# ACMMM2021-Anonymous/video-graph-ssl

Hardware: AMD Instinct MI355X
Metric: pretrain_clips_per_sec (higher is better)
Workload: dtype bf16x6 (fp32 tensors; conv products as 6 bf16 MFMAs on hi/mid/lo splits = fp32-grade, fp32 accumulate; everything else fp32)

## Files before the change

### include/gca_hip.h

```cpp
#ifndef GCA_HIP_H
#define GCA_HIP_H

#include <stdint.h>

#ifdef __cplusplus
extern "C" {
#endif

#define GCA_OK 0
#define GCA_EINVAL (-1)
#define GCA_ELAUNCH (-2)

int gca_version(void);

int gca_conv_halo_occupancy(int tm, int tn, int math, int64_t lds_bytes);

int gca_set_conv_math(int mode);
int gca_get_conv_math(void);

typedef struct {
  int32_t N, C, D, H, W;
  int32_t K;
  int32_t kd, kh, kw;
  int32_t sd, sh, sw;
  int32_t pd, ph, pw;
  int32_t OD, OH, OW;
  int64_t x_batch_stride;
  int32_t tune_fwd_bm, tune_fwd_splits;
  int32_t tune_dgrad_bm, tune_dgrad_splits;
  int32_t tune_wgrad_splits, tune_wgrad_tile;
  int32_t tune_fwd_tail, tune_dgrad_tail;
  int32_t tune_fwd_math, tune_dgrad_math, tune_wgrad_math;
  int32_t tune_fwd_box, tune_dgrad_box;
// ... 1 lines not shown
} gca_conv_geom;

int64_t gca_conv_pack_elems(const gca_conv_geom* g, int which);
int gca_conv_pack(const gca_conv_geom* g, int which, const float* w, float* packed, void* stream);

#define GCA_PACK_JOB_BYTES 128
int64_t gca_conv_pack_jobs_host(const gca_conv_geom* g, int which, const float* w, float* packed, void* jobs_out);
int64_t gca_conv_pack_jobs_finalize_host(void* jobs, int64_t njobs);
int gca_conv_pack_batched(const void* jobs_dev, int64_t njobs, int64_t total_blocks, void* stream);

int64_t gca_conv_table_rows(const gca_conv_geom* g, int which);
int gca_conv_table_build_host(const gca_conv_geom* g, int which, int32_t* table_host );

int64_t gca_conv_fwd_stat_parts(const gca_conv_geom* g);
int gca_conv_kernel_cfg(const gca_conv_geom* g, int which, int32_t* out4);
int64_t gca_conv_pack_layout(const gca_conv_geom* g, int which);
int64_t gca_conv_fwd_ws_bytes(const gca_conv_geom* g);
int gca_conv_fwd(const gca_conv_geom* g, const void* x, const float* wpack, const int32_t* table,
                 const float* bias, void* y, float* stat_sum, float* stat_sq, void* ws, void* stream);

int64_t gca_conv_dgrad_ws_bytes(const gca_conv_geom* g);
int gca_conv_dgrad(const gca_conv_geom* g, const void* dy, const float* wpack, const int32_t* table,
                   void* dx, int accumulate, void* ws, void* stream);

int64_t gca_conv_wgrad_ws_bytes(const gca_conv_geom* g);
int gca_conv_wgrad(const gca_conv_geom* g, const void* x, const void* dy, const int32_t* table,
                   float* dw, int accumulate, void* ws, void* stream);
typedef struct {
  const float* slabs;
  float* dw;
// ... 164 lines not shown
```

### video-graph-ssl_amd/_hip.py

```python
import ctypes as C
import os

import torch

_HERE = os.path.dirname(os.path.abspath(__file__))
LIB_PATH = os.environ.get('GCA_LIB_PATH') or os.path.join(_HERE, 'libgca_hip.so')


class HipLibraryMissing(RuntimeError):
    pass


if not os.path.exists(LIB_PATH):
    raise HipLibraryMissing(
        'libgca_hip.so is not built (%s). Run ./build_hip.sh or __graft_entry__.build(); there is no '
        'CPU fallback for the product path.' % LIB_PATH)
lib = C.CDLL(LIB_PATH)

c_i32, c_i64, c_f32, c_f64, c_vp = C.c_int32, C.c_int64, C.c_float, C.c_double, C.c_void_p


class ConvGeom(C.Structure):
    _fields_ = [(n, c_i32) for n in ('N', 'C', 'D', 'H', 'W', 'K', 'kd', 'kh', 'kw', 'sd', 'sh', 'sw',
                                     'pd', 'ph', 'pw', 'OD', 'OH', 'OW')] + [('x_batch_stride', c_i64)] + \
# ... 2 lines not shown
                                     'tune_fwd_math', 'tune_dgrad_math', 'tune_wgrad_math', 'tune_fwd_box',
                                     'tune_dgrad_box', 'act_f16')]


class PoolGeom(C.Structure):
    _fields_ = [(n, c_i32) for n in ('N', 'C', 'D', 'H', 'W', 'kd', 'kh', 'kw', 'sd', 'sh', 'sw',
                                     'pd', 'ph', 'pw', 'OD', 'OH', 'OW')]


_GP, _PP = C.POINTER(ConvGeom), C.POINTER(PoolGeom)
SIGNATURES = {
    'gca_version': (c_i32, []),
    'gca_conv_halo_occupancy': (c_i32, [c_i32, c_i32, c_i32, c_i64]),
    'gca_set_conv_math': (c_i32, [c_i32]),
    'gca_get_conv_math': (c_i32, []),
    'gca_conv_pack_elems': (c_i64, [_GP, c_i32]),
    'gca_conv_pack': (c_i32, [_GP, c_i32, c_vp, c_vp, c_vp]),
    'gca_conv_table_rows': (c_i64, [_GP, c_i32]),
    'gca_conv_table_build_host': (c_i32, [_GP, c_i32, c_vp]),
    'gca_conv_fwd_stat_parts': (c_i64, [_GP]),
    'gca_conv_kernel_cfg': (c_i32, [_GP, c_i32, c_vp]),
    'gca_conv_pack_layout': (c_i64, [_GP, c_i32]),
    'gca_conv_fwd_ws_bytes': (c_i64, [_GP]),
    'gca_conv_fwd': (c_i32, [_GP, c_vp, c_vp, c_vp, c_vp, c_vp, c_vp, c_vp, c_vp, c_vp]),
    'gca_conv_dgrad_ws_bytes': (c_i64, [_GP]),
    'gca_conv_dgrad': (c_i32, [_GP, c_vp, c_vp, c_vp, c_vp, c_i32, c_vp, c_vp]),
    'gca_conv_wgrad_cfg': (c_i32, [_GP, c_vp]),
    'gca_conv_wgrad_ws_bytes': (c_i64, [_GP]),
    'gca_conv_wgrad': (c_i32, [_GP, c_vp, c_vp, c_vp, c_vp, c_i32, c_vp, c_vp]),
    'gca_bias_grad': (c_i32, [c_vp, c_i64, c_i64, c_i64, c_vp, c_i32, c_vp]),
    'gca_bn_stats': (c_i32, [c_vp, c_i64, c_i64, c_i64, c_vp, c_vp, c_vp, c_i32, c_vp]),
    'gca_bn_stats_parts': (c_i64, [c_i64, c_i64, c_i64]),
    'gca_bn_finalize': (c_i32, [c_vp, c_vp, c_i64, c_i64, c_f64, c_vp, c_vp, c_f32, c_f32, c_vp, c_vp, c_vp,
                                c_vp, c_vp, c_vp, c_vp, c_vp]),
    'gca_bn_train_fwd': (c_i32, [c_vp, c_vp, c_i64, c_i64, c_f64, c_vp, c_vp, c_f32, c_f32, c_vp, c_vp, c_vp,
                                 c_vp, c_vp, c_vp, c_vp, c_vp, c_vp, c_i32, c_i64, c_i64, c_vp, c_i64, c_i32, c_vp]),
# ... 123 lines not shown
```

### video-graph-ssl_amd/csrc/conv3d.hip

```cpp
#include <cstring>
#include <type_traits>
#include "conv_halo.h"

#include <cstdlib>
#include <vector>

using namespace gca_conv;

namespace {


constexpr int LDK = BK + 4;
constexpr int lds_pitch(int math) { return math == 2 ? 28 : (math == 3 ? 12 : LDK); }
constexpr int lds_bufs(int tm, bool vec, int math) { return (math >= 1 || vec || tm >= 4) ? 1 : 2; }
constexpr int cmax(int a, int b) { return a > b ? a : b; }

template <int TM, int BN, int FAST, bool VEC, int MATH, bool H = false>
__device__ __forceinline__ void igemm_tile(
    const void* __restrict__ src, const float* __restrict__ apack, const int2* __restrict__ table,
    const float* __restrict__ bias, void* __restrict__ dst, float* __restrict__ psum,
    float* __restrict__ psq, float* __restrict__ slab, const IgemmParams p, int bid,
    float* __restrict__ As_, float* __restrict__ Bs_, int* __restrict__ taptab) {
  constexpr unsigned ES = H ? 2u : 4u;
  constexpr int BM = 32 * TM, TN = BN / 128;
// ... 765 lines not shown
  pw.accumulate = ip.accumulate;
  pw.src_nstride = (unsigned)ip.src_nstride;
  pw.src_bytes = ip.src_bytes; pw.dst_bytes = ip.dst_bytes;
  const long long pb = (long long)pack_rows(DK) * pw.Kpad * 2;
  pw.pack_bytes = clamp_buf_bytes(pb);
  return true;
}

inline int stem_copy_dwords(int bw) { return (bw + 4) / 2; }
inline int stem_row_bytes(int bw, int sh, int np) { (void)sh; return 4 * np * stem_copy_dwords(bw) * 4; }
inline bool stem_heuristic_on() {
  static int on = -1;
  if (on < 0) { const char* e = getenv("GCA_STEM"); on = (e && e[0] == '0') ? 0 : 1; }
  return on != 0;
}
inline bool stem_geometry(const gca_conv_geom* g, const IgemmParams& p, int math, StemParams& sp) {
  if (math < 1 || math > 3 || g->C > 4 || g->sw != 2 || g->kw > 8 || g->x_batch_stride % 4 != 0) return false;
  if ((long long)g->N * g->OD * g->OH * g->OW < 256 * 32) return false;
  const int np = math == 3 ? 1 : (math == 2 ? 3 : 2);
  const int nrows = g->C * g->kd * g->kh, nsteps = cdiv(nrows, 2);
  double best = 1e300;
  int bb[3] = {0, 0, 0};
  const int wmr = g->K > 64 ? 4 : 2, npos = 512 / wmr;
  for (int pass = 0; pass < 2 && bb[0] == 0; ++pass) {
    const size_t cap = pass == 0 ? (size_t)(76 << 10) : (size_t)(156 << 10);
    for (int bd = 1; bd <= npos; bd *= 2)
      for (int bh = 1; bd * bh <= npos; bh *= 2) {
        const int bw = npos / (bd * bh);
        if (bw < 4 || bw > 64) continue;
        if (bd > 2 * g->OD || bh > 2 * g->OH || bw > 2 * g->OW) continue;
        const int hd = (bd - 1) * g->sd + g->kd, hh = (bh - 1) * g->sh + g->kh, wp = bw + 4;
        const size_t lds = gca_round_up((2 * nsteps + g->C * hd * hh) * 4, 16) + (size_t)g->C * hd * hh * stem_row_bytes(bw, g->sh, np);
        if (lds > cap) continue;
        const double cover = (double)cdiv(g->OD, bd) * bd / g->OD * cdiv(g->OH, bh) * bh / g->OH * cdiv(g->OW, bw) * bw / g->OW;
        const double staging = (double)g->C * hd * hh * 2 * wp / (double)npos;
        const double cost = cover * (1.0 + staging / (double)(nsteps * 8)) * (bw >= 8 ? 1.0 : 1.15);
        if (cost < best) { best = cost; bb[0] = bd; bb[1] = bh; bb[2] = bw; }
      }
  }
  if (bb[0] == 0) return false;
  sp.g = p;
  sp.wm = wmr;
  sp.bd = bb[0]; sp.bh = bb[1]; sp.bw = bb[2]; sp.lbh = ilog2(bb[1]); sp.lbw = ilog2(bb[2]);
  sp.nbd = cdiv(g->OD, sp.bd); sp.nbh = cdiv(g->OH, sp.bh); sp.nbw = cdiv(g->OW, sp.bw);
  sp.hd = (sp.bd - 1) * g->sd + g->kd; sp.hh = (sp.bh - 1) * g->sh + g->kh; sp.wp = sp.bw + 4;
  sp.cd = stem_copy_dwords(sp.bw); sp.hrowb = stem_row_bytes(sp.bw, g->sh, np);
  sp.sd = g->sd; sp.sh = g->sh; sp.pd = g->pd; sp.ph = g->ph; sp.pw = g->pw;
  sp.kd = g->kd; sp.kh = g->kh; sp.kw = g->kw;
  sp.nrows = nrows; sp.nsteps = nsteps;
  sp.Mrows = pack_rows(g->K);
  sp.rowoff_bytes = (int)gca_round_up((2 * nsteps + g->C * sp.hd * sp.hh) * 4, 16);
  sp.cs_bytes = (unsigned)((long long)g->D * g->H * g->W * (g->act_f16 ? 2 : 4));
  const long long pb = (long long)nsteps * sp.Mrows * (math == 3 ? 32 : (math == 2 ? 96 : 64));
  sp.pack_bytes = clamp_buf_bytes(pb);
  sp.m_w2 = gca_make_magic((unsigned)sp.wp); sp.m_hdh = gca_make_magic((unsigned)(sp.hd * sp.hh));
  sp.m_hh = gca_make_magic((unsigned)sp.hh);
  return true;
// ... 46 lines not shown
                           ((double)c.q[0] * c.q[1] * c.q[2]);
      const double cost = cover * (1.0 + 0.08 * hp.P / bn) * (w >= 8 ? 1.0 : (w >= 4 ? 1.1 : 1.3));
      if (cost < best) { best = cost; bd = d; bh = h; bw = w; }
    }
  cost_out = best;
  return best < 1e299;
}

inline IgemmCfg cfg_for(const gca_conv_geom* g, int which, const ClassInfo& c, const IgemmParams& p, size_t nclasses) {
  int fbm, fs, tail, box;
  tune_of(g, which, fbm, fs, tail, box);
  const int math = resolve_math(which == 0 ? g->tune_fwd_math : g->tune_dgrad_math, g->act_f16);
  if (which == 0 && ((fbm & 4096) || (fbm == 0 && stem_heuristic_on()))) {
    StemParams sp;
    if (stem_geometry(g, p, math, sp))
      return IgemmCfg{32 * sp.wm, 512 / sp.wm, 1, sp.nsteps, 0, 0, math, ConvKernel::Stem, sp.bd, sp.bh, sp.bw, math == 3};
  }
  if (fbm & 4096) { fbm = 0; fs = 0; tail = 0; }
  if ((fbm & 8192) || (fbm == 0 && pw_heuristic_on())) {
    PwParams pw;
    if (pw_geometry(g, which, p, pw)) return IgemmCfg{128, 128, 1, pw.Kpad / 32, 0, 0, 3, ConvKernel::Pointwise, 0, 0, 0, 1};
  }
  if (fbm & 8192) { fbm = 0; fs = 0; tail = 0; }
  {
    int bd = box & 255, bh = (box >> 8) & 255, bw = (box >> 16) & 255, rows = fbm & 1023;
    bool use = false;
    HaloParams hp;
    if ((fbm & 2048) && !(fbm & (4096 | 8192))) {
      use = bd > 0 && halo_geometry(c, p, bd, bh, bw, math, hp);
    } else if (fbm == 0 && halo_heuristic_on() && (c.ntaps >= 3 || math == 3) && c.srcC >= 32 && p.Ntot >= 128LL * 192) {
      double cost = 0, cost2 = 0;
// ... 54 lines not shown
  else
    hipLaunchKernelGGL((conv_igemm_kernel<TM, BN, FAST, VEC, 0>), grid, dim3(256), 0, st, src, apack, table, bias,
                       dst, psum, psq, slab, p);
}

template <int TM>
void launch_tm(const IgemmCfg& c, int fast, dim3 grid, hipStream_t st, const float* src, const float* apack,
               const int2* table, const float* bias, float* dst, float* psum, float* psq, float* slab,
               const IgemmParams& p) {
  if (c.bn == 256) launch_one<TM, 256, 1, true>(c.math, grid, st, src, apack, table, bias, dst, psum, psq, slab, p, c.h);
  else if (fast == 1) launch_one<TM, 128, 1, false>(c.math, grid, st, src, apack, table, bias, dst, psum, psq, slab, p, c.h);
  else if (fast == 2) launch_one<TM, 128, 2, false>(c.math, grid, st, src, apack, table, bias, dst, psum, psq, slab, p, c.h);
  else launch_one<TM, 128, 0, false>(c.math, grid, st, src, apack, table, bias, dst, psum, psq, slab, p, c.h);
}

inline int stat_parts(const IgemmCfg& c, long long Ntot, long long halo_tiles = 0) {
  if (c.splits > 1) return (int)gca_ceil_div(Ntot, FINISH_CHUNK);
  if (c.kernel != ConvKernel::Gather) return (int)halo_tiles;
  return (int)gca_ceil_div(Ntot, c.bn);
}

int finish_slabs(const IgemmCfg& c, const float* slab, const float* bias, float* dst, float* psum, float* psq, const IgemmParams& p,
                 hipStream_t st) {
  const dim3 grid((unsigned)p.DK, (unsigned)p.P);
  if (c.h)
    hipLaunchKernelGGL(conv_splitk_finish_kernel<_Float16>, grid, dim3(256), 0, st, slab, c.splits, bias,
                       reinterpret_cast<_Float16*>(dst), psum, psq, p);
  else
    hipLaunchKernelGGL(conv_splitk_finish_kernel<float>, grid, dim3(256), 0, st, slab, c.splits, bias, dst, psum, psq, p);
  return gca_launch_status();
}

// ... 78 lines not shown
  return finish_slabs(cf, slab, bias, dst, psum, psq, p, st);
}

int run_class_pw(const gca_conv_geom* g, int which, const float* src, const float* apack, const float* bias, float* dst, float* psum,
                 float* psq, const IgemmParams& p, hipStream_t st) {
  PwParams pw;
  if (!pw_geometry(g, which, p, pw)) return GCA_EINVAL;
  return pw_launch(pw, src, reinterpret_cast<const unsigned char*>(apack), bias, dst, psum, psq, st);
}

int run_class_stem(const gca_conv_geom* g, const IgemmCfg& cf, const float* src, const float* apack, const float* bias, float* dst,
                   float* psum, float* psq, const IgemmParams& p, hipStream_t st) {
  StemParams sp;
  if (!stem_geometry(g, p, cf.math, sp) || sp.bd != cf.bd || sp.bh != cf.bh || sp.bw != cf.bw) return GCA_EINVAL;
  sp.g.splits = 1; sp.g.kt_per_split = sp.nsteps;
  sp.g.tilesM = cdiv(p.DK, 32 * sp.wm);
  const long long tn = (long long)g->N * sp.nbd * sp.nbh * sp.nbw;
  if (tn > 0x7fffffffLL) return GCA_EINVAL;
  sp.g.tilesN = (int)tn; sp.g.tileN_off = 0;
  sp.g.P = (int)tn;
  return stem_launch(cf.math, sp, src, reinterpret_cast<const unsigned char*>(apack), bias, dst, psum, psq, st);
}

struct ConvLaunch {
  std::vector<ClassInfo> cls;
  std::vector<IgemmParams> p;
  std::vector<IgemmCfg> cf;
};

ConvLaunch resolve_launch(const gca_conv_geom* g, int which) {
  ConvLaunch L;
  build_classes(g, which, L.cls);
  const size_t n = L.cls.size();
  L.p.assign(n, IgemmParams{});
  L.cf.assign(n, IgemmCfg{});
// ... 42 lines not shown
  }
  return g_conv_math;
}
}

extern "C" {

int gca_version(void) { return 15; }

int gca_set_conv_math(int mode) {
  if (mode < 0 || mode > 2) return GCA_EINVAL;
  g_conv_math = mode;
  return GCA_OK;
}
int gca_get_conv_math(void) { return conv_math(); }

int64_t gca_conv_pack_elems(const gca_conv_geom* g, int which) {
  if (!geom_ok(g) || (which != 0 && which != 1)) return GCA_EINVAL;
  int64_t n = 0;
  for (const ClassInfo& c : resolve_launch(g, which).cls) n += pack_reserve(c);
  return n > 0 ? n : 64;
}

static void pack_params_of(const gca_conv_geom* g, int which, const ClassInfo& c, const IgemmCfg& cf, PackParams& p) {
  const int T = taps(g);
  p.fmt = (int)cf.kernel; p.math = cf.math; p.SC = c.srcC;
  p.nsteps = cf.kernel == ConvKernel::Stem ? cf.kt_per_split : cdiv(c.srcC, 16) * c.ntaps;
  const bool pwfmt = p.fmt == 3;
  p.Kred = (int)c.Kred; p.M = c.M; p.Kpad = pwfmt ? (int)gca_round_up(c.srcC, 32) : (int)c.Kpad; p.Mrows = pack_rows(c.M);
  p.ntaps = p.fmt == 2 ? g->kd * g->kh : c.ntaps; p.nb = c.nb; p.nc = c.nc;
// ... 142 lines not shown
int gca_conv_kernel_cfg(const gca_conv_geom* g, int which, int32_t* out4) {
  if (!geom_ok(g) || which < 0 || which > 1 || !out4) return GCA_EINVAL;
  const ConvLaunch L = resolve_launch(g, which);
  for (size_t i = 0; i < L.cls.size(); ++i) {
    const ClassInfo& c = L.cls[i];
    const IgemmCfg& cf = L.cf[i];
    if (c.ntaps == 0) continue;
    out4[0] = cf.bm; out4[1] = cf.bn; out4[2] = cf.splits;
    out4[3] = (int)L.cls.size() | (fast_of(c.ntaps) << 8) | (c.vec << 10) | (cf.math << 12) | ((cf.kernel == ConvKernel::Halo) << 14) |
              (cf.h << 15) | ((cf.kernel == ConvKernel::Stem) << 16) | ((cf.kernel == ConvKernel::Pointwise) << 17);
    return GCA_OK;
  }
  return GCA_EINVAL;
}

int64_t gca_conv_fwd_stat_parts(const gca_conv_geom* g) {
  if (!geom_ok(g)) return GCA_EINVAL;
  const ConvLaunch L = resolve_launch(g, 0);
  const IgemmCfg& cf = L.cf[0];
  if (cf.kernel == ConvKernel::Pointwise) return (int64_t)g->N * cdiv((int)((long long)g->OD * g->OH * g->OW), 128);
  return stat_parts(cf, L.p[0].Ntot, cf.kernel != ConvKernel::Gather ? halo_tiles_n(g, L.cls[0], cf) : 0);
}

int64_t gca_conv_fwd_ws_bytes(const gca_conv_geom* g) { return geom_ok(g) ? ws_bytes_for(g, 0) : GCA_EINVAL; }
int64_t gca_conv_dgrad_ws_bytes(const gca_conv_geom* g) { return geom_ok(g) ? ws_bytes_for(g, 1) : GCA_EINVAL; }

int gca_conv_fwd(const gca_conv_geom* g, const void* x_, const float* wpack, const int32_t* table,
                 const float* bias, void* y_, float* stat_sum, float* stat_sq, void* ws, void* stream) {
  const float* x = reinterpret_cast<const float*>(x_);
  float* y = reinterpret_cast<float*>(y_);
// ... 70 lines not shown
```

### video-graph-ssl_amd/csrc/conv3d_stem.hip

```cpp
#include <cstring>
#include "conv_igemm_host.h"
#include "conv_halo.h"

using namespace gca_conv;

namespace {

constexpr int rowb(int math) { return math == 3 ? 32 : (math == 2 ? 96 : 64); }
constexpr int nparts(int math) { return math == 3 ? 1 : (math == 2 ? 3 : 2); }
__device__ __forceinline__ unsigned short f16_bits(float v) { return __builtin_bit_cast(unsigned short, (_Float16)v); }

template <int MATH, int WM>
__global__ __launch_bounds__(256, 2) void conv_stem_kernel(
    const void* __restrict__ src, const unsigned char* __restrict__ apack, const float* __restrict__ bias,
    void* __restrict__ dst, float* __restrict__ psum, float* __restrict__ psq, const StemParams sp) {
  static_assert(MATH >= 1 && MATH <= 3, "bf16x3 / bf16x6 / fp16 storage");
  constexpr bool F16 = MATH == 3;
  constexpr unsigned ES = F16 ? 2u : 4u;
  static_assert(WM == 2 || WM == 4, "wave grid");
  constexpr int WN = 4 / WM, BM = 32 * WM, TN = 4;
  constexpr int ROWB = rowb(MATH), NP = nparts(MATH);
  const IgemmParams& p = sp.g;
  extern __shared__ __attribute__((aligned(16))) unsigned char smem[];
  int* const rowoff = reinterpret_cast<int*>(smem);
  unsigned* const rowbase = reinterpret_cast<unsigned*>(smem) + 2 * sp.nsteps;
  unsigned char* const Hs = smem + sp.rowoff_bytes;

  const int tid = threadIdx.x, lane = tid & 63, wave = tid >> 6, wm = wave / WN, wn = wave % WN, lh = lane >> 5, ll = lane & 31;
  int bid = gca_xcd_remap(blockIdx.x, gridDim.x);
  const int tileM = bid % p.tilesM, tileN = bid / p.tilesM;
  const int per_img = sp.nbd * sp.nbh * sp.nbw;
  const int img = tileN / per_img;
  int tb = tileN - img * per_img;
  const int tbd = tb / (sp.nbh * sp.nbw); tb -= tbd * (sp.nbh * sp.nbw);
  const int tbh = tb / sp.nbw, tbw = tb - tbh * sp.nbw;
  const int q0d = tbd * sp.bd, q0h = tbh * sp.bh, q0w = tbw * sp.bw;

  const int wp = sp.wp;
  const unsigned COPYB = (unsigned)sp.cd * 4u, PARTB = 2u * COPYB, PHASEB = PARTB * NP, HROWB = (unsigned)sp.hrowb;
  const int khd = sp.kd * sp.kh;
  for (int r = tid; r < 2 * sp.nsteps; r += 256) {
    int off = 0;
    if (r < sp.nrows) {
      const int c = r / khd, ab = r - c * khd, a = ab / sp.kh, b = ab - a * sp.kh;
      off = ((c * sp.hd + a) * sp.hh + b) * (int)HROWB;
    }
    rowoff[r] = off;
  }

  const __amdgpu_buffer_rsrc_t ra = __builtin_amdgcn_make_buffer_rsrc(const_cast<unsigned char*>(apack), 0, sp.pack_bytes, 0x00020000);
  const unsigned avoff = (unsigned)(tileM * BM + 32 * wm + ll) * ROWB + (unsigned)lh * 16u;
  const unsigned astep = (unsigned)sp.Mrows * ROWB;
  float4 afn[NP];
  auto a_issue = [&](int s) __attribute__((always_inline)) {
#pragma unroll
    for (int q = 0; q < NP; ++q) {
      const f32x4 f = __builtin_bit_cast(f32x4, __builtin_amdgcn_raw_buffer_load_b128(ra, (int)(avoff + 32u * q), (int)((unsigned)s * astep), 0));
      afn[q] = make_float4(f.x, f.y, f.z, f.w);
    }
  };
  a_issue(0);

  {
    const __amdgpu_buffer_rsrc_t rs = __builtin_amdgcn_make_buffer_rsrc(const_cast<void*>(src), 0, p.src_bytes, 0x00020000);
    const int nhrows = p.SC * sp.hd * sp.hh;
    const int s0d = q0d * sp.sd - sp.pd, s0h = q0h * sp.sh - sp.ph, s0w = q0w * 2 - sp.pw;
    const unsigned ibase = (unsigned)((long long)img * p.src_nstride);
    const int hdh = sp.hd * sp.hh;
    for (int hr = tid; hr < nhrows; hr += 256) {
      const int c = (int)gca_fdiv((unsigned)hr, sp.m_hdh), rem = hr - c * hdh;
      const int zd = (int)gca_fdiv((unsigned)rem, sp.m_hh), zh = rem - zd * sp.hh;
      const int id = s0d + zd, ih = s0h + zh;
      const bool ok = (unsigned)id < (unsigned)p.SD && (unsigned)ih < (unsigned)p.SH;
      rowbase[hr] = ok ? (ibase + (unsigned)((id * p.SH + ih) * p.SW)) * ES + (unsigned)c * sp.cs_bytes : 0xffffffffu;
    }
// ... 39 lines not shown
          unsigned h, l;
          split_bf16x2(v[k][0], v[k][1], h, l);
          *reinterpret_cast<unsigned*>(d) = h; *reinterpret_cast<unsigned*>(d + PARTB) = l;
          split_bf16x2(v[k][1], v[k][2], h, l);
          *reinterpret_cast<unsigned*>(d + COPYB) = h; *reinterpret_cast<unsigned*>(d + COPYB + PARTB) = l;
        }
      }
    }
  }

  unsigned bpos[TN];
  bool cval[TN];
  int cq[TN][3];
#pragma unroll
  for (int j = 0; j < TN; ++j) {
    const int cidx = wn * 128 + j * 32 + ll;
    const int zw = cidx & (sp.bw - 1), t1 = cidx >> sp.lbw;
    const int zh = t1 & (sp.bh - 1), zd = t1 >> sp.lbh;
    cq[j][0] = q0d + zd; cq[j][1] = q0h + zh; cq[j][2] = q0w + zw;
    cval[j] = cq[j][0] < p.QD && cq[j][1] < p.QH && cq[j][2] < p.QW;
    bpos[j] = (unsigned)((zd * sp.sd) * sp.hh + zh * sp.sh) * HROWB + (unsigned)(zw & 1) * COPYB + (unsigned)(zw & ~1) * 2u;
  }

  f32x16 acc[TN];
#pragma unroll
  for (int j = 0; j < TN; ++j)
#pragma unroll
    for (int r = 0; r < 16; ++r) acc[j][r] = 0.f;

  auto load_b = [&](float4 (&bf)[NP], int j, unsigned ro) __attribute__((always_inline)) {
    const unsigned char* bp = Hs + bpos[j] + ro;
#pragma unroll
    for (int q = 0; q < NP; ++q) {
      const unsigned* e = reinterpret_cast<const unsigned*>(bp + q * PARTB);
      const unsigned* o = reinterpret_cast<const unsigned*>(bp + PHASEB + q * PARTB);
      bf[q] = make_float4(__uint_as_float(e[0]), __uint_as_float(e[1]), __uint_as_float(o[0]), __uint_as_float(o[1]));
    }
  };
  auto mma = [&](f32x16& c, const float4 (&af)[NP], const float4 (&bf)[NP]) __attribute__((always_inline)) {
    if constexpr (MATH == 3) {
      c = __builtin_amdgcn_mfma_f32_32x32x16_f16(__builtin_bit_cast(f16x8, af[0]), __builtin_bit_cast(f16x8, bf[0]), c, 0, 0, 0);
    } else {
      const bf16x8 xh = __builtin_bit_cast(bf16x8, af[0]), xl = __builtin_bit_cast(bf16x8, af[NP - 1]);
// ... 7 lines not shown
        c = __builtin_amdgcn_mfma_f32_32x32x16_bf16(xh, ym, c, 0, 0, 0);
      } else {
        c = __builtin_amdgcn_mfma_f32_32x32x16_bf16(xl, yh, c, 0, 0, 0);
        c = __builtin_amdgcn_mfma_f32_32x32x16_bf16(xh, yl, c, 0, 0, 0);
      }
      c = __builtin_amdgcn_mfma_f32_32x32x16_bf16(xh, yh, c, 0, 0, 0);
    }
  };

  __syncthreads();
  unsigned ro = (unsigned)rowoff[lh];
  float4 bfc[NP], bfn[NP];
  load_b(bfc, 0, ro);
  for (int s = 0; s < sp.nsteps; ++s) {
    const unsigned ro_next = (unsigned)rowoff[2 * min(s + 1, sp.nsteps - 1) + lh];
    float4 af[NP];
#pragma unroll
    for (int q = 0; q < NP; ++q) af[q] = afn[q];
    a_issue(min(s + 1, sp.nsteps - 1));
#pragma unroll
    for (int j = 0; j < TN; ++j) {
      if (j + 1 < TN) load_b(bfn, j + 1, ro); else load_b(bfn, 0, ro_next);
      mma(acc[j], af, bfc);
#pragma unroll
      for (int q = 0; q < NP; ++q) bfc[q] = bfn[q];
    }
    ro = ro_next;
  }
  __syncthreads();

  const int mbase = tileM * BM + 32 * wm;
  const int rows_left = p.DK - mbase - 4 * lh;
  const int DHW = p.DH * p.DW;
  const unsigned DSP = (unsigned)(p.DD * DHW);
  const unsigned rowb_ = DSP * ES;
  const __amdgpu_buffer_rsrc_t rd = __builtin_amdgcn_make_buffer_rsrc(dst, 0, p.dst_bytes, 0x00020000);
#pragma unroll
  for (int j = 0; j < TN; ++j) {
    const unsigned dsp = (unsigned)(cq[j][0] * DHW + cq[j][1] * p.DW + cq[j][2]);
    const unsigned vb = cval[j] ? (((unsigned)img * (unsigned)p.DK + (unsigned)(mbase + 4 * lh)) * DSP + dsp) * ES : 0xffffffffu;
#pragma unroll
    for (int r = 0; r < 16; ++r) {
      const int rr = (r & 3) + 8 * (r >> 2);
      const unsigned vo = rr < rows_left ? vb : 0xffffffffu;
      float v = acc[j][r];
      if (bias) v += bias[min(mbase + rr + 4 * lh, p.DK - 1)];
      if (F16) __builtin_amdgcn_raw_buffer_store_b16(f16_bits(v), rd, (int)vo, (int)((unsigned)rr * rowb_), 0);
      else __builtin_amdgcn_raw_buffer_store_b32(__float_as_uint(v), rd, (int)vo, (int)((unsigned)rr * rowb_), 0);
    }
  }
  if (psum) {
    float* red = reinterpret_cast<float*>(Hs);
#pragma unroll
    for (int r = 0; r < 16; ++r) {
      float sm = 0.f, sq = 0.f;
#pragma unroll
      for (int j = 0; j < TN; ++j) { const float v = cval[j] ? acc[j][r] : 0.f; sm += v; sq += v * v; }
      sm = half_wave_sum_hi(sm);
      sq = half_wave_sum_hi(sq);
      const int rr = 32 * wm + (r & 3) + 8 * (r >> 2) + 4 * lh;
      if (ll == 31) { red[(wn * BM + rr) * 2] = sm; red[(wn * BM + rr) * 2 + 1] = sq; }
    }
    __syncthreads();
    if (tid < BM && tileM * BM + tid < p.DK) {
      float sm = red[tid * 2], sq = red[tid * 2 + 1];
      if (WN == 2) { sm += red[(BM + tid) * 2]; sq += red[(BM + tid) * 2 + 1]; }
      const long long m = tileM * BM + tid;
      psum[m * p.P + tileN] = sm;
      psq[m * p.P + tileN] = sq;
    }
  }
}

}

namespace gca_conv {

size_t stem_lds_bytes(const StemParams& sp, int math) {
  const size_t halo = (size_t)sp.g.SC * sp.hd * sp.hh * sp.hrowb;
  return (size_t)sp.rowoff_bytes + (halo > 2048 ? halo : 2048);
}

int stem_launch(int math, const StemParams& sp, const void* src, const unsigned char* apack, const float* bias, void* dst,
                float* psum, float* psq, hipStream_t st) {
  const size_t lds = stem_lds_bytes(sp, math);
  const long long nblk = (long long)sp.g.tilesM * sp.g.tilesN;
  if (nblk <= 0 || nblk > 0x7fffffffLL || lds > (size_t)(160 << 10) - 1024) return GCA_EINVAL;
  static bool raised[4][2] = {};
#define GCA_SK2(M, W)                                                                                                      \
  {                                                                                                                        \
    if (lds > (48u << 10) && !raised[M][W / 4]) {                                                                          \
      if (hipFuncSetAttribute(reinterpret_cast<const void*>(&conv_stem_kernel<M, W>),                                      \
                              hipFuncAttributeMaxDynamicSharedMemorySize, 160 << 10) != hipSuccess) return GCA_ELAUNCH;   \
      raised[M][W / 4] = true;                                                                                             \
    }                                                                                                                      \
    hipLaunchKernelGGL((conv_stem_kernel<M, W>), dim3((unsigned)nblk), dim3(256), lds, st, src, apack, bias, dst, psum, psq, sp); \
  }
#define GCA_SK(M) { if (sp.wm == 4) GCA_SK2(M, 4) else GCA_SK2(M, 2) }
  switch (math) {
    case 1: GCA_SK(1) break;
    case 2: GCA_SK(2) break;
    case 3: GCA_SK(3) break;
    default: return GCA_EINVAL;
  }
#undef GCA_SK
#undef GCA_SK2
  return gca_launch_status();
}

}
```

### video-graph-ssl_amd/csrc/conv_halo.h

```cpp
#pragma once
#include "conv_igemm_host.h"

namespace gca_conv {

struct HaloParams {
  IgemmParams g;
  int bd, bh, bw;
  int lbh, lbw;
  int hd, hh, hw;
  int h0d, h0h, h0w;
  int dmin_d, dmin_h, dmin_w;
  int nbd, nbh, nbw;
  int P;
  int nchunks, chunks_per_split;
  int Mrows;
  unsigned cs_bytes;
  unsigned pack_bytes;
  const float* in_scale;
  const float* in_shift;
};

struct HaloCfg {
  int bm, bn;
  int bd, bh, bw;
  int splits, chunks_per_split;
  int math;
};

struct StemParams {
  IgemmParams g;
  int wm;
  int bd, bh, bw, lbh, lbw;
  int nbd, nbh, nbw;
  int hd, hh;
  int wp;
  int cd, hrowb;
  int sd, sh, pd, ph, pw;
  int kd, kh, kw;
  int nrows, nsteps;
  int Mrows;
  int rowoff_bytes;
  unsigned cs_bytes;
  unsigned pack_bytes;
  gca_magic m_w2, m_hdh, m_hh;
};

// ... 85 lines not shown
```

### video-graph-ssl_amd/engine/ops.py

```python
import ctypes as C
import functools
import os

import torch

from .. import _hip as H
from .._hip import aptr, is_half, ptr, stream
from . import tune
from .tune import TUNE_HALO, TUNE_PW, TUNE_STEM, TUNE_VEC

F32 = torch.float32
F16 = torch.float16


def _t3(v):
    return (v, v, v) if isinstance(v, int) else tuple(int(a) for a in v)


class _Workspace:

    def __init__(self):
        self.buf = {}
        self.captured = set()
        self.retired = []
# ... 26 lines not shown
_TUNE_DIRTY = [False]
_TUNE_PATH = os.environ.get('GCA_TUNE_CACHE', '')


CONV_MATH = {'f32': 0, 'bf16x3': 1, 'bf16x6': 2}
ACT_F16 = [False]


def set_conv_math(mode):
    ACT_F16[0] = mode == 'fp16'
    H.call('gca_set_conv_math', CONV_MATH['bf16x6' if mode == 'fp16' else mode])


def get_conv_math():
    return 'fp16' if ACT_F16[0] else ('f32', 'bf16x3', 'bf16x6')[H.lib.gca_get_conv_math()]


def cast_f16(x):
    rows, re = (1, x.numel()) if x.is_contiguous() else (x.shape[0], x[0].numel())
    if not x.is_contiguous() and not x[0].is_contiguous():
        raise RuntimeError('only channel slices of a contiguous (N, Ctot, ...) buffer are supported')
    y = torch.empty(x.shape, dtype=F16, device=x.device)
    H.call('gca_cast_f16', ptr(x), rows, re, re if x.is_contiguous() else x.stride(0), aptr(y), stream())
    return y


def load_tune_cache(path):
    import json
    with open(path) as f:
        for k, v in json.load(f).items():
# ... 75 lines not shown
        out = (C.c_int32 * 4)()
        if which == 2:
            H.call('gca_conv_wgrad_cfg', self.gp, out)
        else:
            H.call('gca_conv_kernel_cfg', self.gp, which, out)
        return tuple(out)

    WGRAD_KERNELS = {11: 'temporal32', 12: 'temporal64', 13: 'spatial', 14: 'stem'}
    WGRAD_SHAPES = tune.WGRAD_SHAPES

    def kernel(self, which):
        kc = self.cfg(which)[3]
        if which == 2:
            return self.WGRAD_KERNELS.get(kc & 255, 'gather')
        return next((name for name, _, bit in _KERNELS if kc >> bit & 1), 'gather')

    def math(self, which):
        return self.cfg(which)[3] >> 12 & 3

    def pack_layout(self, which):
        return 0 if which == 2 else H.lib.gca_conv_pack_layout(self.gp, which)

    def tune_key(self, which):
        g = self.g
        geom = (g.N, g.C, g.D, g.H, g.W, g.K, g.kd, g.kh, g.kw, g.sd, g.sh, g.sw, g.pd, g.ph, g.pw, g.x_batch_stride)
        return 'v%d%s:%d:%s' % (H.lib.gca_version(), 'h' if g.act_f16 else ('', 'b', 'c')[H.lib.gca_get_conv_math()], which,
                                ','.join(str(int(v)) for v in geom))

    def set_code(self, which, code):
        for field, v in zip(code._fields, code):
# ... 700 lines not shown
```

Baseline: 1670.

## Add register-blocked stem conv tile computing two M sub-tiles per wave

Adds an RT=2 variant of the stem conv kernel where each wave holds two 32-row M sub-tiles of accumulators and reuses each loaded B fragment for two MFMAs. For bf16x6 with K>64 it uses WM=2,RT=2 over 256 positions, and for fp16 it uses WM=1,RT=2. This halves B-fragment LDS reads per MFMA. BN-stat partial reduction is reworked to match, with per-half partials and an LDS exchange. It is enabled by default through GCA_STEM_RB, and it raises register pressure and changes the stat-part count layout.

```diff
diff --git a/include/gca_hip.h b/include/gca_hip.h
--- a/include/gca_hip.h
+++ b/include/gca_hip.h
@@ -17,6 +17,9 @@
 
 int gca_set_conv_math(int mode);
 int gca_get_conv_math(void);
+
+int gca_set_stem_rb(int on);
+int gca_get_stem_rb(void);
 
 typedef struct {
   int32_t N, C, D, H, W;
@@ -48,6 +51,7 @@
 
 int64_t gca_conv_fwd_stat_parts(const gca_conv_geom* g);
 int gca_conv_kernel_cfg(const gca_conv_geom* g, int which, int32_t* out4);
+int gca_conv_stem_shape(const gca_conv_geom* g, int32_t* out4);
 int64_t gca_conv_pack_layout(const gca_conv_geom* g, int which);
 int64_t gca_conv_fwd_ws_bytes(const gca_conv_geom* g);
 int gca_conv_fwd(const gca_conv_geom* g, const void* x, const float* wpack, const int32_t* table,
diff --git a/video-graph-ssl_amd/_hip.py b/video-graph-ssl_amd/_hip.py
--- a/video-graph-ssl_amd/_hip.py
+++ b/video-graph-ssl_amd/_hip.py
@@ -40,12 +40,15 @@
     'gca_conv_halo_occupancy': (c_i32, [c_i32, c_i32, c_i32, c_i64]),
     'gca_set_conv_math': (c_i32, [c_i32]),
     'gca_get_conv_math': (c_i32, []),
+    'gca_set_stem_rb': (c_i32, [c_i32]),
+    'gca_get_stem_rb': (c_i32, []),
     'gca_conv_pack_elems': (c_i64, [_GP, c_i32]),
     'gca_conv_pack': (c_i32, [_GP, c_i32, c_vp, c_vp, c_vp]),
     'gca_conv_table_rows': (c_i64, [_GP, c_i32]),
     'gca_conv_table_build_host': (c_i32, [_GP, c_i32, c_vp]),
     'gca_conv_fwd_stat_parts': (c_i64, [_GP]),
     'gca_conv_kernel_cfg': (c_i32, [_GP, c_i32, c_vp]),
+    'gca_conv_stem_shape': (c_i32, [_GP, c_vp]),
     'gca_conv_pack_layout': (c_i64, [_GP, c_i32]),
     'gca_conv_fwd_ws_bytes': (c_i64, [_GP]),
     'gca_conv_fwd': (c_i32, [_GP, c_vp, c_vp, c_vp, c_vp, c_vp, c_vp, c_vp, c_vp, c_vp]),
diff --git a/video-graph-ssl_amd/csrc/conv3d.hip b/video-graph-ssl_amd/csrc/conv3d.hip
--- a/video-graph-ssl_amd/csrc/conv3d.hip
+++ b/video-graph-ssl_amd/csrc/conv3d.hip
@@ -803,33 +803,48 @@
   if (on < 0) { const char* e = getenv("GCA_STEM"); on = (e && e[0] == '0') ? 0 : 1; }
   return on != 0;
 }
+int g_stem_rb = -1;
+inline bool stem_rb_on() {
+  if (g_stem_rb < 0) { const char* e = getenv("GCA_STEM_RB"); g_stem_rb = (e && e[0] == '0') ? 0 : 1; }
+  return g_stem_rb != 0;
+}
+inline bool stem_pick_box(const gca_conv_geom* g, int npos, int np, int nsteps, size_t cap, int (&bb)[3]) {
+  double best = 1e300;
+  bb[0] = 0;
+  for (int bd = 1; bd <= npos; bd *= 2)
+    for (int bh = 1; bd * bh <= npos; bh *= 2) {
+      const int bw = npos / (bd * bh);
+      if (bw < 4 || bw > 64) continue;
+      if (bd > 2 * g->OD || bh > 2 * g->OH || bw > 2 * g->OW) continue;
+      const int hd = (bd - 1) * g->sd + g->kd, hh = (bh - 1) * g->sh + g->kh, wp = bw + 4;
+      const size_t lds = gca_round_up((2 * nsteps + g->C * hd * hh) * 4, 16) + (size_t)g->C * hd * hh * stem_row_bytes(bw, g->sh, np);
+      if (lds > cap) continue;
+      const double cover = (double)cdiv(g->OD, bd) * bd / g->OD * cdiv(g->OH, bh) * bh / g->OH * cdiv(g->OW, bw) * bw / g->OW;
+      const double staging = (double)g->C * hd * hh * 2 * wp / (double)npos;
+      const double cost = cover * (1.0 + staging / (double)(nsteps * 8)) * (bw >= 8 ? 1.0 : 1.15);
+      if (cost < best) { best = cost; bb[0] = bd; bb[1] = bh; bb[2] = bw; }
+    }
+  return bb[0] != 0;
+}
 inline bool stem_geometry(const gca_conv_geom* g, const IgemmParams& p, int math, StemParams& sp) {
   if (math < 1 || math > 3 || g->C > 4 || g->sw != 2 || g->kw > 8 || g->x_batch_stride % 4 != 0) return false;
   if ((long long)g->N * g->OD * g->OH * g->OW < 256 * 32) return false;
   const int np = math == 3 ? 1 : (math == 2 ? 3 : 2);
   const int nrows = g->C * g->kd * g->kh, nsteps = cdiv(nrows, 2);
-  double best = 1e300;
   int bb[3] = {0, 0, 0};
-  const int wmr = g->K > 64 ? 4 : 2, npos = 512 / wmr;
-  for (int pass = 0; pass < 2 && bb[0] == 0; ++pass) {
-    const size_t cap = pass == 0 ? (size_t)(76 << 10) : (size_t)(156 << 10);
-    for (int bd = 1; bd <= npos; bd *= 2)
-      for (int bh = 1; bd * bh <= npos; bh *= 2) {
-        const int bw = npos / (bd * bh);
-        if (bw < 4 || bw > 64) continue;
-        if (bd > 2 * g->OD || bh > 2 * g->OH || bw > 2 * g->OW) continue;
-        const int hd = (bd - 1) * g->sd + g->kd, hh = (bh - 1) * g->sh + g->kh, wp = bw + 4;
-        const size_t lds = gca_round_up((2 * nsteps + g->C * hd * hh) * 4, 16) + (size_t)g->C * hd * hh * stem_row_bytes(bw, g->sh, np);
-        if (lds > cap) continue;
-        const double cover = (double)cdiv(g->OD, bd) * bd / g->OD * cdiv(g->OH, bh) * bh / g->OH * cdiv(g->OW, bw) * bw / g->OW;
-        const double staging = (double)g->C * hd * hh * 2 * wp / (double)npos;
-        const double cost = cover * (1.0 + staging / (double)(nsteps * 8)) * (bw >= 8 ? 1.0 : 1.15);
-        if (cost < best) { best = cost; bb[0] = bd; bb[1] = bh; bb[2] = bw; }
-      }
-  }
-  if (bb[0] == 0) return false;
+  const bool rb = stem_rb_on();
+  int wmr = g->K > 64 ? 4 : 2, rt = 1;
+  if (g->K > 64) {
+    if (rb && math == 2 && stem_pick_box(g, 256, np, nsteps, (size_t)(76 << 10), bb)) { wmr = 2; rt = 2; }
+    else if (!stem_pick_box(g, 128, np, nsteps, (size_t)(76 << 10), bb) && !stem_pick_box(g, 128, np, nsteps, (size_t)(156 << 10), bb))
+      return false;
+  } else {
+    if (!stem_pick_box(g, 256, np, nsteps, (size_t)(76 << 10), bb) && !stem_pick_box(g, 256, np, nsteps, (size_t)(156 << 10), bb))
+      return false;
+    if (rb && math == 3) { wmr = 1; rt = 2; }
+  }
   sp.g = p;
-  sp.wm = wmr;
+  sp.wm = wmr; sp.rt = rt;
   sp.bd = bb[0]; sp.bh = bb[1]; sp.bw = bb[2]; sp.lbh = ilog2(bb[1]); sp.lbw = ilog2(bb[2]);
   sp.nbd = cdiv(g->OD, sp.bd); sp.nbh = cdiv(g->OH, sp.bh); sp.nbw = cdiv(g->OW, sp.bw);
   sp.hd = (sp.bd - 1) * g->sd + g->kd; sp.hh = (sp.bh - 1) * g->sh + g->kh; sp.wp = sp.bw + 4;
@@ -906,7 +921,7 @@
   if (which == 0 && ((fbm & 4096) || (fbm == 0 && stem_heuristic_on()))) {
     StemParams sp;
     if (stem_geometry(g, p, math, sp))
-      return IgemmCfg{32 * sp.wm, 512 / sp.wm, 1, sp.nsteps, 0, 0, math, ConvKernel::Stem, sp.bd, sp.bh, sp.bw, math == 3};
+      return IgemmCfg{32 * sp.wm * sp.rt, sp.wm * sp.rt == 4 ? 128 : 256, 1, sp.nsteps, 0, 0, math, ConvKernel::Stem, sp.bd, sp.bh, sp.bw, math == 3};
   }
   if (fbm & 4096) { fbm = 0; fs = 0; tail = 0; }
   if ((fbm & 8192) || (fbm == 0 && pw_heuristic_on())) {
@@ -991,8 +1006,11 @@
   else launch_one<TM, 128, 0, false>(c.math, grid, st, src, apack, table, bias, dst, psum, psq, slab, p, c.h);
 }
 
+inline int stem_parts_per_box(const IgemmCfg& c) { return c.bd * c.bh * c.bw / c.bn; }
+
 inline int stat_parts(const IgemmCfg& c, long long Ntot, long long halo_tiles = 0) {
   if (c.splits > 1) return (int)gca_ceil_div(Ntot, FINISH_CHUNK);
+  if (c.kernel == ConvKernel::Stem) return (int)halo_tiles * stem_parts_per_box(c);
   if (c.kernel != ConvKernel::Gather) return (int)halo_tiles;
   return (int)gca_ceil_div(Ntot, c.bn);
 }
@@ -1101,11 +1119,11 @@
   StemParams sp;
   if (!stem_geometry(g, p, cf.math, sp) || sp.bd != cf.bd || sp.bh != cf.bh || sp.bw != cf.bw) return GCA_EINVAL;
   sp.g.splits = 1; sp.g.kt_per_split = sp.nsteps;
-  sp.g.tilesM = cdiv(p.DK, 32 * sp.wm);
+  sp.g.tilesM = cdiv(p.DK, 32 * sp.wm * sp.rt);
   const long long tn = (long long)g->N * sp.nbd * sp.nbh * sp.nbw;
-  if (tn > 0x7fffffffLL) return GCA_EINVAL;
+  if (tn > 0x3fffffffLL) return GCA_EINVAL;
   sp.g.tilesN = (int)tn; sp.g.tileN_off = 0;
-  sp.g.P = (int)tn;
+  sp.g.P = (int)tn * stem_parts_per_box(cf);
   return stem_launch(cf.math, sp, src, reinterpret_cast<const unsigned char*>(apack), bias, dst, psum, psq, st);
 }
 
@@ -1178,6 +1196,13 @@
   return GCA_OK;
 }
 int gca_get_conv_math(void) { return conv_math(); }
+
+int gca_set_stem_rb(int on) {
+  if (on < 0 || on > 1) return GCA_EINVAL;
+  g_stem_rb = on;
+  return GCA_OK;
+}
+int gca_get_stem_rb(void) { return stem_rb_on() ? 1 : 0; }
 
 int64_t gca_conv_pack_elems(const gca_conv_geom* g, int which) {
   if (!geom_ok(g) || (which != 0 && which != 1)) return GCA_EINVAL;
@@ -1350,6 +1375,15 @@
   return GCA_EINVAL;
 }
 
+int gca_conv_stem_shape(const gca_conv_geom* g, int32_t* out4) {
+  if (!geom_ok(g) || !out4) return GCA_EINVAL;
+  const ConvLaunch L = resolve_launch(g, 0);
+  StemParams sp;
+  if (L.cf.empty() || L.cf[0].kernel != ConvKernel::Stem || !stem_geometry(g, L.p[0], L.cf[0].math, sp)) return GCA_EINVAL;
+  out4[0] = 32 * sp.wm * sp.rt; out4[1] = sp.bd * sp.bh * sp.bw; out4[2] = sp.wm; out4[3] = sp.rt;
+  return GCA_OK;
+}
+
 int64_t gca_conv_fwd_stat_parts(const gca_conv_geom* g) {
   if (!geom_ok(g)) return GCA_EINVAL;
   const ConvLaunch L = resolve_launch(g, 0);
diff --git a/video-graph-ssl_amd/csrc/conv3d_stem.hip b/video-graph-ssl_amd/csrc/conv3d_stem.hip
--- a/video-graph-ssl_amd/csrc/conv3d_stem.hip
+++ b/video-graph-ssl_amd/csrc/conv3d_stem.hip
@@ -10,15 +10,17 @@
 constexpr int nparts(int math) { return math == 3 ? 1 : (math == 2 ? 3 : 2); }
 __device__ __forceinline__ unsigned short f16_bits(float v) { return __builtin_bit_cast(unsigned short, (_Float16)v); }
 
-template <int MATH, int WM>
+template <int MATH, int WM, int RT>
 __global__ __launch_bounds__(256, 2) void conv_stem_kernel(
     const void* __restrict__ src, const unsigned char* __restrict__ apack, const float* __restrict__ bias,
     void* __restrict__ dst, float* __restrict__ psum, float* __restrict__ psq, const StemParams sp) {
   static_assert(MATH >= 1 && MATH <= 3, "bf16x3 / bf16x6 / fp16 storage");
   constexpr bool F16 = MATH == 3;
   constexpr unsigned ES = F16 ? 2u : 4u;
-  static_assert(WM == 2 || WM == 4, "wave grid");
-  constexpr int WN = 4 / WM, BM = 32 * WM, TN = 4;
+  static_assert((RT == 1 && (WM == 2 || WM == 4)) || (RT == 2 && (WM == 1 || WM == 2)), "wave grid");
+  constexpr int WN = 4 / WM, BM = 32 * WM * RT, BN = WM == 4 ? 128 : 256, TN = BN / (32 * WN);
+  constexpr bool XCH = WN == 4;
+  constexpr bool PER_HALF = WM == 2 && RT == 2;
   constexpr int ROWB = rowb(MATH), NP = nparts(MATH);
   const IgemmParams& p = sp.g;
   extern __shared__ __attribute__((aligned(16))) unsigned char smem[];
@@ -49,16 +51,26 @@
   }
 
   const __amdgpu_buffer_rsrc_t ra = __builtin_amdgcn_make_buffer_rsrc(const_cast<unsigned char*>(apack), 0, sp.pack_bytes, 0x00020000);
-  const unsigned avoff = (unsigned)(tileM * BM + 32 * wm + ll) * ROWB + (unsigned)lh * 16u;
+  const int mbase = tileM * BM + 32 * RT * wm;
+  const bool on1 = RT == 2 && mbase + 32 < p.DK;
+  const unsigned avoff = (unsigned)(mbase + ll) * ROWB + (unsigned)lh * 16u;
   const unsigned astep = (unsigned)sp.Mrows * ROWB;
-  float4 afn[NP];
+  float4 afn[RT][NP];
   auto a_issue = [&](int s) __attribute__((always_inline)) {
 #pragma unroll
-    for (int q = 0; q < NP; ++q) {
-      const f32x4 f = __builtin_bit_cast(f32x4, __builtin_amdgcn_raw_buffer_load_b128(ra, (int)(avoff + 32u * q), (int)((unsigned)s * astep), 0));
-      afn[q] = make_float4(f.x, f.y, f.z, f.w);
+    for (int i = 0; i < RT; ++i) {
+      if (i == 1 && !on1) continue;
+#pragma unroll
+      for (int q = 0; q < NP; ++q) {
+        const f32x4 f = __builtin_bit_cast(f32x4, __builtin_amdgcn_raw_buffer_load_b128(ra, (int)(avoff + 32u * ROWB * i + 32u * q), (int)((unsigned)s * astep), 0));
+        afn[i][q] = make_float4(f.x, f.y, f.z, f.w);
+      }
     }
   };
+  if (RT == 2) {
+#pragma unroll
+    for (int q = 0; q < NP; ++q) afn[RT - 1][q] = make_float4(0.f, 0.f, 0.f, 0.f);
+  }
   a_issue(0);
 
   {
@@ -128,7 +140,7 @@
   int cq[TN][3];
 #pragma unroll
   for (int j = 0; j < TN; ++j) {
-    const int cidx = wn * 128 + j * 32 + ll;
+    const int cidx = wn * (32 * TN) + j * 32 + ll;
     const int zw = cidx & (sp.bw - 1), t1 = cidx >> sp.lbw;
     const int zh = t1 & (sp.bh - 1), zd = t1 >> sp.lbh;
     cq[j][0] = q0d + zd; cq[j][1] = q0h + zh; cq[j][2] = q0w + zw;
@@ -136,11 +148,13 @@
     bpos[j] = (unsigned)((zd * sp.sd) * sp.hh + zh * sp.sh) * HROWB + (unsigned)(zw & 1) * COPYB + (unsigned)(zw & ~1) * 2u;
   }
 
-  f32x16 acc[TN];
-#pragma unroll
-  for (int j = 0; j < TN; ++j)
-#pragma unroll
-    for (int r = 0; r < 16; ++r) acc[j][r] = 0.f;
+  f32x16 acc[RT][TN];
+#pragma unroll
+  for (int i = 0; i < RT; ++i)
+#pragma unroll
+    for (int j = 0; j < TN; ++j)
+#pragma unroll
+      for (int r = 0; r < 16; ++r) acc[i][j][r] = 0.f;
 
   auto load_b = [&](float4 (&bf)[NP], int j, unsigned ro) __attribute__((always_inline)) {
     const unsigned char* bp = Hs + bpos[j] + ro;
@@ -178,14 +192,17 @@
   load_b(bfc, 0, ro);
   for (int s = 0; s < sp.nsteps; ++s) {
     const unsigned ro_next = (unsigned)rowoff[2 * min(s + 1, sp.nsteps - 1) + lh];
-    float4 af[NP];
-#pragma unroll
-    for (int q = 0; q < NP; ++q) af[q] = afn[q];
+    float4 af[RT][NP];
+#pragma unroll
+    for (int i = 0; i < RT; ++i)
+#pragma unroll
+      for (int q = 0; q < NP; ++q) af[i][q] = afn[i][q];
     a_issue(min(s + 1, sp.nsteps - 1));
 #pragma unroll
     for (int j = 0; j < TN; ++j) {
       if (j + 1 < TN) load_b(bfn, j + 1, ro); else load_b(bfn, 0, ro_next);
-      mma(acc[j], af, bfc);
+      mma(acc[0][j], af[0], bfc);
+      if (RT == 2 && on1) mma(acc[RT - 1][j], af[RT - 1], bfc);
 #pragma unroll
       for (int q = 0; q < NP; ++q) bfc[q] = bfn[q];
     }
@@ -193,42 +210,76 @@
   }
   __syncthreads();
 
-  const int mbase = tileM * BM + 32 * wm;
-  const int rows_left = p.DK - mbase - 4 * lh;
   const int DHW = p.DH * p.DW;
   const unsigned DSP = (unsigned)(p.DD * DHW);
   const unsigned rowb_ = DSP * ES;
   const __amdgpu_buffer_rsrc_t rd = __builtin_amdgcn_make_buffer_rsrc(dst, 0, p.dst_bytes, 0x00020000);
 #pragma unroll
-  for (int j = 0; j < TN; ++j) {
-    const unsigned dsp = (unsigned)(cq[j][0] * DHW + cq[j][1] * p.DW + cq[j][2]);
-    const unsigned vb = cval[j] ? (((unsigned)img * (unsigned)p.DK + (unsigned)(mbase + 4 * lh)) * DSP + dsp) * ES : 0xffffffffu;
-#pragma unroll
-    for (int r = 0; r < 16; ++r) {
-      const int rr = (r & 3) + 8 * (r >> 2);
-      const unsigned vo = rr < rows_left ? vb : 0xffffffffu;
-      float v = acc[j][r];
-      if (bias) v += bias[min(mbase + rr + 4 * lh, p.DK - 1)];
-      if (F16) __builtin_amdgcn_raw_buffer_store_b16(f16_bits(v), rd, (int)vo, (int)((unsigned)rr * rowb_), 0);
-      else __builtin_amdgcn_raw_buffer_store_b32(__float_as_uint(v), rd, (int)vo, (int)((unsigned)rr * rowb_), 0);
+  for (int i = 0; i < RT; ++i) {
+    if (i == 1 && !on1) continue;
+    const int mb = mbase + 32 * i;
+    const int rows_left = p.DK - mb - 4 * lh;
+#pragma unroll
+    for (int j = 0; j < TN; ++j) {
+      const unsigned dsp = (unsigned)(cq[j][0] * DHW + cq[j][1] * p.DW + cq[j][2]);
+      const unsigned vb = cval[j] ? (((unsigned)img * (unsigned)p.DK + (unsigned)(mb + 4 * lh)) * DSP + dsp) * ES : 0xffffffffu;
+#pragma unroll
+      for (int r = 0; r < 16; ++r) {
+        const int rr = (r & 3) + 8 * (r >> 2);
+        const unsigned vo = rr < rows_left ? vb : 0xffffffffu;
+        float v = acc[i][j][r];
+        if (bias) v += bias[min(mb + rr + 4 * lh, p.DK - 1)];
+        if (F16) __builtin_amdgcn_raw_buffer_store_b16(f16_bits(v), rd, (int)vo, (int)((unsigned)rr * rowb_), 0);
+        else __builtin_amdgcn_raw_buffer_store_b32(__float_as_uint(v), rd, (int)vo, (int)((unsigned)rr * rowb_), 0);
+      }
     }
   }
   if (psum) {
+#pragma clang fp contract(off)
+    constexpr int NH = XCH ? 2 : WN;
     float* red = reinterpret_cast<float*>(Hs);
-#pragma unroll
-    for (int r = 0; r < 16; ++r) {
-      float sm = 0.f, sq = 0.f;
-#pragma unroll
-      for (int j = 0; j < TN; ++j) { const float v = cval[j] ? acc[j][r] : 0.f; sm += v; sq += v * v; }
-      sm = half_wave_sum_hi(sm);
-      sq = half_wave_sum_hi(sq);
-      const int rr = 32 * wm + (r & 3) + 8 * (r >> 2) + 4 * lh;
-      if (ll == 31) { red[(wn * BM + rr) * 2] = sm; red[(wn * BM + rr) * 2 + 1] = sq; }
-    }
-    __syncthreads();
-    if (tid < BM && tileM * BM + tid < p.DK) {
+    float* xch = red + 512;
+#pragma unroll
+    for (int i = 0; i < RT; ++i) {
+      const int half = XCH ? wn >> 1 : wn;
+      const bool first = !XCH || !(wn & 1);
+      if (XCH && first) {
+#pragma unroll
+        for (int r = 0; r < 16; ++r) {
+          float sm = 0.f, sq = 0.f;
+#pragma unroll
+          for (int j = 0; j < TN; ++j) { const float v = cval[j] ? acc[i][j][r] : 0.f; sm += v; sq += v * v; }
+          xch[((half * 16 + r) * 2) * 64 + lane] = sm;
+          xch[((half * 16 + r) * 2 + 1) * 64 + lane] = sq;
+        }
+      }
+      if (XCH) __syncthreads();
+      if (!XCH || !first) {
+#pragma unroll
+        for (int r = 0; r < 16; ++r) {
+          float sm = 0.f, sq = 0.f;
+          if (XCH) { sm = xch[((half * 16 + r) * 2) * 64 + lane]; sq = xch[((half * 16 + r) * 2 + 1) * 64 + lane]; }
+#pragma unroll
+          for (int j = 0; j < TN; ++j) { const float v = cval[j] ? acc[i][j][r] : 0.f; sm += v; sq += v * v; }
+          sm = half_wave_sum_hi(sm);
+          sq = half_wave_sum_hi(sq);
+          const int rr = 32 * (RT * wm + i) + (r & 3) + 8 * (r >> 2) + 4 * lh;
+          if (ll == 31) { red[(half * BM + rr) * 2] = sm; red[(half * BM + rr) * 2 + 1] = sq; }
+        }
+      }
+      if (XCH) __syncthreads();
+    }
+    if (!XCH) __syncthreads();
+    if (PER_HALF) {
+      const int h = tid >> 7, r = tid & 127;
+      if (tileM * BM + r < p.DK) {
+        const long long m = tileM * BM + r;
+        psum[m * p.P + 2 * tileN + h] = red[(h * BM + r) * 2];
+        psq[m * p.P + 2 * tileN + h] = red[(h * BM + r) * 2 + 1];
+      }
+    } else if (tid < BM && tileM * BM + tid < p.DK) {
       float sm = red[tid * 2], sq = red[tid * 2 + 1];
-      if (WN == 2) { sm += red[(BM + tid) * 2]; sq += red[(BM + tid) * 2 + 1]; }
+      if (NH == 2) { sm += red[(BM + tid) * 2]; sq += red[(BM + tid) * 2 + 1]; }
       const long long m = tileM * BM + tid;
       psum[m * p.P + tileN] = sm;
       psq[m * p.P + tileN] = sq;
@@ -242,7 +293,8 @@
 
 size_t stem_lds_bytes(const StemParams& sp, int math) {
   const size_t halo = (size_t)sp.g.SC * sp.hd * sp.hh * sp.hrowb;
-  return (size_t)sp.rowoff_bytes + (halo > 2048 ? halo : 2048);
+  const size_t scratch = sp.wm == 1 ? 2048 + 16384 : 2048;
+  return (size_t)sp.rowoff_bytes + (halo > scratch ? halo : scratch);
 }
 
 int stem_launch(int math, const StemParams& sp, const void* src, const unsigned char* apack, const float* bias, void* dst,
@@ -250,21 +302,26 @@
   const size_t lds = stem_lds_bytes(sp, math);
   const long long nblk = (long long)sp.g.tilesM * sp.g.tilesN;
   if (nblk <= 0 || nblk > 0x7fffffffLL || lds > (size_t)(160 << 10) - 1024) return GCA_EINVAL;
-  static bool raised[4][2] = {};
-#define GCA_SK2(M, W)                                                                                                      \
+  static bool raised[4][4] = {};
+#define GCA_SK2(M, W, R)                                                                                                   \
   {                                                                                                                        \
-    if (lds > (48u << 10) && !raised[M][W / 4]) {                                                                          \
-      if (hipFuncSetAttribute(reinterpret_cast<const void*>(&conv_stem_kernel<M, W>),                                      \
+    if (lds > (48u << 10) && !raised[M][2 * (R - 1) + (W > 3 - R)]) {                                                   \
+      if (hipFuncSetAttribute(reinterpret_cast<const void*>(&conv_stem_kernel<M, W, R>),                                   \
                               hipFuncAttributeMaxDynamicSharedMemorySize, 160 << 10) != hipSuccess) return GCA_ELAUNCH;   \
-      raised[M][W / 4] = true;                                                                                             \
+      raised[M][2 * (R - 1) + (W > 3 - R)] = true;                                                                               \
     }                                                                                                                      \
-    hipLaunchKernelGGL((conv_stem_kernel<M, W>), dim3((unsigned)nblk), dim3(256), lds, st, src, apack, bias, dst, psum, psq, sp); \
-  }
-#define GCA_SK(M) { if (sp.wm == 4) GCA_SK2(M, 4) else GCA_SK2(M, 2) }
+    hipLaunchKernelGGL((conv_stem_kernel<M, W, R>), dim3((unsigned)nblk), dim3(256), lds, st, src, apack, bias, dst, psum, psq, sp); \
+  }
+#define GCA_SK(M, W2, W1)                                                                                                  \
+  {                                                                                                                        \
+    if (sp.rt == 1) { if (sp.wm == 4) GCA_SK2(M, 4, 1) else if (sp.wm == 2) GCA_SK2(M, 2, 1) else return GCA_EINVAL; }     \
+    else if (sp.rt == 2) { if (sp.wm == 2) W2 else if (sp.wm == 1) W1 else return GCA_EINVAL; }                            \
+    else return GCA_EINVAL;                                                                                                \
+  }
   switch (math) {
-    case 1: GCA_SK(1) break;
-    case 2: GCA_SK(2) break;
-    case 3: GCA_SK(3) break;
+    case 1: GCA_SK(1, return GCA_EINVAL;, return GCA_EINVAL;) break;
+    case 2: GCA_SK(2, GCA_SK2(2, 2, 2), return GCA_EINVAL;) break;
+    case 3: GCA_SK(3, return GCA_EINVAL;, GCA_SK2(3, 1, 2)) break;
     default: return GCA_EINVAL;
   }
 #undef GCA_SK
diff --git a/video-graph-ssl_amd/csrc/conv_halo.h b/video-graph-ssl_amd/csrc/conv_halo.h
--- a/video-graph-ssl_amd/csrc/conv_halo.h
+++ b/video-graph-ssl_amd/csrc/conv_halo.h
@@ -29,7 +29,7 @@
 
 struct StemParams {
   IgemmParams g;
-  int wm;
+  int wm, rt;
   int bd, bh, bw, lbh, lbw;
   int nbd, nbh, nbw;
   int hd, hh;
diff --git a/video-graph-ssl_amd/engine/ops.py b/video-graph-ssl_amd/engine/ops.py
--- a/video-graph-ssl_amd/engine/ops.py
+++ b/video-graph-ssl_amd/engine/ops.py
@@ -64,6 +64,14 @@
 
 def get_conv_math():
     return 'fp16' if ACT_F16[0] else ('f32', 'bf16x3', 'bf16x6')[H.lib.gca_get_conv_math()]
+
+
+def set_stem_rb(on):
+    H.call('gca_set_stem_rb', int(bool(on)))
+
+
+def get_stem_rb():
+    return bool(H.lib.gca_get_stem_rb())
 
 
 def cast_f16(x):
@@ -169,6 +177,11 @@
         if which == 2:
             return self.WGRAD_KERNELS.get(kc & 255, 'gather')
         return next((name for name, _, bit in _KERNELS if kc >> bit & 1), 'gather')
+
+    def stem_shape(self):
+        out = (C.c_int32 * 4)()
+        H.call('gca_conv_stem_shape', self.gp, out)
+        return tuple(out)
 
     def math(self, which):
         return self.cfg(which)[3] >> 12 & 3
```

Result: no change. 1673 (median of 2 runs) (+0.2%).
